# Jarvis73/PEMP

Hardware: AMD Instinct MI355X
Metric: episodes/sec (PEMP stage-1 eval step, PASCAL-5i-shaped 1-shot, ResNet-50) (higher is better)
Workload: dtype f32

## Files before the change

include/pemp_hip.h:

```cpp
#ifndef PEMP_HIP_H
#define PEMP_HIP_H

#include <stddef.h>
#include <stdint.h>

#ifdef __cplusplus
extern "C" {
#endif

#define PEMP_ABI_VERSION 2

#define PEMP_CONV_RELU 1u
#define PEMP_CONV_SHIFT_PER_IMAGE 2u
#define PEMP_CONV_STEM4 4u
#define PEMP_CONV_POOL3S2 8u
#define PEMP_CONV_OUT_SPLIT3 16u
#define PEMP_CONV_IN_SPLIT3 32u
#define PEMP_CONV_OUT_SPLIT3_ALSO 64u

typedef struct pemp_conv_desc {
    int32_t N, H, W;
    int32_t Cin, ldx;
    int32_t Ho, Wo;
    int32_t Cout, ldy;
// ... 13 lines not shown
int pemp_conv2d_nhwc_f32(const pemp_conv_desc* d, const float* x, const float* w, float* y,
                         const float* scale, const float* shift, const float* residual,
                         void* stream);

int pemp_conv2d_padv_nhwc_f32(const pemp_conv_desc* d, const float* x, const float* w, float* y,
                              const float* scale, const float* shift, const float* residual,
                              const float* pad_value, void* stream);

int pemp_conv2d_hybrid_rows(const pemp_conv_desc* d);

int pemp_conv2d_group_nhwc_f32(int n, const pemp_conv_desc* d, const float* const* x, const float* const* w,
                               float* const* y, const float* const* scale, const float* const* shift,
                               const float* const* residual, const float* const* pad_value, void* stream);

int pemp_pack_split3_bf16(const float* w, void* out, int cout, int kpad, void* stream);

int pemp_conv2d_bf16_nhwc(const pemp_conv_desc* d, const void* x, const void* w, void* y, const float* scale,
                          const float* shift, const void* residual, const void* pad_value, int out_f32, void* stream);
int pemp_convert_f32_bf16(const float* x, void* y, long long n, void* stream);
int pemp_convert_bf16_f32(const void* x, float* y, long long n, void* stream);

int pemp_conv2d_dropblock_nhwc_f32(const pemp_conv_desc* d, const float* x, const float* w, float* y, const float* scale,
                                   const float* shift, const float* residual, const float* rowmask, const int* kept_count,
                                   void* ws, size_t ws_bytes, void* stream);
int pemp_bn_apply_dropblock_f32(const float* z, int ldz, const float* mean, const float* invstd, const float* gamma,
                                const float* beta, float* y, int ldy, int M, int C, const float* rowmask,
                                const int* kept_count, void* stream);

int pemp_pack_input_nhwc4_f32(const float* img, const float* prior, float* out,
                              int N, int H, int W, void* stream);
// ... 254 lines not shown
```

pemp_amd/_lib.py:

```python
import ctypes as C
import os

import torch

_HERE = os.path.dirname(os.path.abspath(__file__))
LIB_PATH = os.environ.get("PEMP_HIP_LIB", os.path.join(_HERE, "libpemp_hip.so"))

c_fp = C.c_void_p
c_int = C.c_int
c_size = C.c_size_t


class ConvDesc(C.Structure):
    _fields_ = [(n, C.c_int32) for n in
                ("N", "H", "W", "Cin", "ldx", "Ho", "Wo", "Cout", "ldy", "KH", "KW",
                 "stride", "pad", "dil", "ldr", "Kpad")] + [("flags", C.c_uint32), ("tile", C.c_int32)]


class SampleDesc(C.Structure):
    _fields_ = [("img_off", C.c_int64), ("msk_off", C.c_int64), ("img_out", C.c_int64), ("msk_out", C.c_int64)] + \
               [(n, C.c_int32) for n in ("hs", "ws", "sh", "sw", "oy", "ox", "flip", "jitter_order")] + \
               [("jitter", C.c_float * 3), ("mask_mode", C.c_int32), ("ksx", C.c_int32), ("ksy", C.c_int32),
                ("ws_off", C.c_int64)]

# ... 5 lines not shown
CONV_OUT_SPLIT3 = 16
CONV_IN_SPLIT3 = 32
CONV_OUT_SPLIT3_ALSO = 64

SYMBOLS = {
    "pemp_last_error": (C.c_char_p, []),
    "pemp_abi_version": (c_int, []),
    "pemp_conv2d_hybrid_rows": (c_int, [C.POINTER(ConvDesc)]),
    "pemp_conv2d_tile_shape": (c_int, [c_int, C.POINTER(c_int), C.POINTER(c_int)]),
    "pemp_conv2d_nhwc_f32": (c_int, [C.POINTER(ConvDesc), c_fp, c_fp, c_fp, c_fp, c_fp, c_fp, c_fp]),
    "pemp_conv2d_padv_splitk_nhwc_f32": (c_int, [C.POINTER(ConvDesc), c_fp, c_fp, c_fp, c_fp, c_fp, c_fp, c_fp, c_fp, c_size, c_fp]),
    "pemp_conv2d_padv_nhwc_f32": (c_int, [C.POINTER(ConvDesc), c_fp, c_fp, c_fp, c_fp, c_fp, c_fp, c_fp, c_fp]),
    "pemp_conv2d_group_nhwc_f32": (c_int, [c_int, C.POINTER(ConvDesc)] + [C.POINTER(c_fp)] * 7 + [c_fp]),
    "pemp_conv2d_bf16_nhwc": (c_int, [C.POINTER(ConvDesc), c_fp, c_fp, c_fp, c_fp, c_fp, c_fp, c_fp, c_int, c_fp]),
    "pemp_pack_split3_bf16": (c_int, [c_fp, c_fp, c_int, c_int, c_fp]),
    "pemp_convert_f32_bf16": (c_int, [c_fp, c_fp, C.c_longlong, c_fp]),
    "pemp_convert_bf16_f32": (c_int, [c_fp, c_fp, C.c_longlong, c_fp]),
    "pemp_conv2d_dropblock_nhwc_f32": (c_int, [C.POINTER(ConvDesc), c_fp, c_fp, c_fp, c_fp, c_fp, c_fp, c_fp, c_fp, c_fp, c_size, c_fp]),
    "pemp_bn_apply_dropblock_f32": (c_int, [c_fp, c_int, c_fp, c_fp, c_fp, c_fp, c_fp, c_int, c_int, c_int, c_fp, c_fp, c_fp]),
    "pemp_pack_input_nhwc4_f32": (c_int, [c_fp, c_fp, c_fp, c_int, c_int, c_int, c_fp]),
    "pemp_maxpool2d_nhwc_f32": (c_int, [c_fp, c_fp] + [c_int] * 11 + [c_fp]),
    "pemp_global_avgpool_nhwc_f32": (c_int, [c_fp, c_fp, c_int, c_int, c_int, c_int, c_fp]),
    "pemp_channel_affine_multi_f32": (c_int, [c_fp, c_int, c_int, c_int, c_int,
                                              C.POINTER(c_fp), C.POINTER(c_fp), C.POINTER(c_fp),
                                              C.POINTER(c_int), c_fp]),
    "pemp_mpm_workspace_bytes": (c_size, [c_int] * 5),
    "pemp_mpm_protos_f32": (c_int, [c_fp, c_int, c_fp, c_fp, c_fp, c_fp, c_size] + [c_int] * 8 + [c_fp]),
    "pemp_map_workspace_bytes": (c_size, [c_int] * 4),
    "pemp_masked_avg_pool_f32": (c_int, [c_fp, c_int, c_fp, c_fp, c_fp, c_size] + [c_int] * 8 + [c_fp]),
    "pemp_cosine_proto_max_f32": (c_int, [c_fp, c_int, c_fp, c_fp, c_fp, c_int, c_int, c_int, c_int,
# ... 140 lines not shown
```

pemp_amd/csrc/conv_common.h:

```cpp
#pragma once
#include "common.h"

namespace pemp {

typedef __attribute__((ext_vector_type(16))) float f32x16;
typedef __attribute__((ext_vector_type(4))) float v4f;
typedef __attribute__((ext_vector_type(8))) __bf16 bf16x8;
typedef __attribute__((ext_vector_type(2))) unsigned int u32x2;

#define PEMP_CONV_BF16_IO 0x100u

__device__ __forceinline__ v4f load_quad(const float* base, size_t off, unsigned bf16) {
    if (!bf16) return *(const v4f*)(base + off);
    const u32x2 r = *(const u32x2*)((const unsigned short*)base + off);
    return v4f{__builtin_bit_cast(float, r.x << 16), __builtin_bit_cast(float, r.x & 0xFFFF0000u),
               __builtin_bit_cast(float, r.y << 16), __builtin_bit_cast(float, r.y & 0xFFFF0000u)};
}

__device__ __forceinline__ unsigned int bf16_bits(float f) {
    const unsigned int u = __builtin_bit_cast(unsigned int, f);
    if ((u & 0x7FFFFFFFu) > 0x7F800000u) return (u >> 16) | 0x40u;
    return (u + 0x7FFFu + ((u >> 16) & 1u)) >> 16;
}

// ... 300 lines not shown
int conv_dma2_hybrid_rows(int M, int Cout);
int launch_conv_dma2_bf16(int shape, const ConvArgs& a, hipStream_t st);
int launch_conv_dma2_db(int shape, ConvArgs a, void* ws, size_t ws_bytes, bool split, hipStream_t st);
struct SplitKPlan { int full, split, pieces; size_t ws_bytes; };
SplitKPlan conv_dma2_splitk_plan(int shape, const ConvArgs& a);
int launch_conv_dma2_splitk(int shape, ConvArgs a, void* ws, size_t ws_bytes, hipStream_t st);
int launch_conv_dma2_split3(int shape, ConvArgs a, void* ws, size_t ws_bytes, bool split, hipStream_t st);
int launch_conv_dma2_group_split3(int shape, ConvGroupArgs& g, hipStream_t st);
int launch_conv_dma2_split3_stats(int shape, const ConvArgs& a, hipStream_t st);
bool conv_dma2_split3_stats_shape(int shape);
int launch_conv_dma2_split3_persist(int shape, const ConvArgs& a, hipStream_t st);
bool conv_dma2_persist_out_split3(int shape);
int launch_conv_dma2_split3_pre(int shape, bool persistent, const ConvArgs& a, hipStream_t st);
bool conv_panel_supported(const ConvArgs& a);
int launch_conv_panel(int shape, const ConvArgs& a, hipStream_t st);
int conv_dma2_simds();
int pack_split3(const float* w, void* out, int cout, int kpad, hipStream_t st);
int launch_conv_stem_pool(const ConvArgs& a, hipStream_t st);
int conv_stem_pool_out(int i);

}
```

pemp_amd/csrc/conv_igemm.hip:

```cpp
#include "conv_tiles.h"

namespace pemp {


template <int BM, int BN, int WGM, bool STEM>
__global__ __launch_bounds__(256) void conv_igemm_kernel(ConvArgs a) {
    constexpr int WGN = 4 / WGM;
    constexpr int WM = BM / WGM, WN = BN / WGN;
    constexpr int TM = WM / 32, TN = WN / 32;
    constexpr int AL = BM / 32, BL = BN / 32;
    static_assert(TM >= 1 && TN >= 1, "wave tile");

    extern __shared__ __attribute__((aligned(16))) v4f smem[];
    v4f* As = smem;
    v4f* Bs = smem + 2 * 8 * BM;

    const int tid = threadIdx.x;
    const int lane = tid & 63;
    const int wave = tid >> 6;
    const int wm0 = (wave / WGN) * WM;
    const int wn0 = (wave % WGN) * WN;
    const int lr = lane & 31, lh = lane >> 5;

    const int ntn = a.Cout / BN;
// ... 336 lines not shown
        if (conv_dma2_supported(a)) {
            PEMP_REQUIRE_COUT("conv2d", t.shape, a.Cout);
            return launch_conv_dma2(t.shape, a, st);
        }
        t.family = TILE_DMA;
        if (t.shape == 8) t.shape = 3;
    }
    if (t.family == TILE_DMA) {
        PEMP_REQUIRE_COUT("conv2d", t.shape, a.Cout);
        return launch_conv_dma(t.shape, a, st);
    }
    PEMP_REQUIRE(t.shape != 1 || a.Cout % 128 == 0, "conv2d: tile 128x128 needs Cout %% 128 == 0");
    return launch_conv(t.shape, a, st);
}


extern "C" int pemp_conv2d_group_nhwc_f32(int n, const pemp_conv_desc* d, const float* const* x, const float* const* w,
                                          float* const* y, const float* const* scale, const float* const* shift,
                                          const float* const* residual, const float* const* pad_value, void* stream) {
    PEMP_REQUIRE(n >= 1 && n <= CONV_GROUP_MAX && d && x && w && y, "conv2d_group: 1..%d member convs", CONV_GROUP_MAX);
    ConvGroupArgs g;
    g.n = n;
    const int tile = d[0].tile;
    const TileId t = decode_tile(tile);
    const bool s3 = t.family == TILE_SPLIT3 && t.exists && !t.splitk && !t.persistent && !t.panel && !t.presplit;
    PEMP_REQUIRE((t.family == TILE_DMA2 && !t.splitk && t.shape <= 8) || s3, "conv2d_group: tile must be one of the buffer-addressed variants 21..28 or 41..44, 46, got %d", tile);
    for (int i = 0; i < n; ++i) {
        PEMP_REQUIRE(d[i].tile == tile, "conv2d_group: every member must name the same tile variant");
        PEMP_REQUIRE(!pad_value || (pad_value[i] != nullptr) == (pad_value[0] != nullptr), "conv2d_group: pad_value for every member or for none");
        const int rc = conv_fill(&d[i], x[i], w[i], y[i], scale ? scale[i] : nullptr, shift ? shift[i] : nullptr,
// ... 208 lines not shown
```

pemp_amd/csrc/conv_panel.hip:

```cpp
#include "conv_tiles.h"

namespace pemp {

typedef __attribute__((address_space(3))) void* lptr_t;
typedef __attribute__((ext_vector_type(4))) unsigned int v4u;

template <int NK> constexpr bool panel_early() { return NK >= 4; }
template <int NK, int BN> constexpr bool panel_two_blocks() { return BN == 64 && NK <= 4; }
template <int NK, int BN> constexpr int panel_stages() {
    if (!panel_early<NK>()) return 3;
    if (NK == 4) return 5;
    return BN == 64 ? 8 : 6;
}
template <int NK, int NS, int BL, int NST>
constexpr int panel_behind(int kt) {
    int c = 0;
    for (int u = kt + 1 - NS; u <= kt - 1; ++u) {
        const int ku = ((u % NK) + NK) % NK;
        if (u > kt + 1 - NS) c += BL;
        if (ku == NK - 1) c += NST;
    }
    return c;
}
template <int NK, int NS, int BL, int NST>
constexpr int panel_behind_max() {
    int m = 0;
    for (int kt = 0; kt < NK; ++kt) m = panel_behind<NK, NS, BL, NST>(kt) > m ? panel_behind<NK, NS, BL, NST>(kt) : m;
    return m;
}
template <int NK, int NS, int BL, int NST, int KT = 0>
__device__ __forceinline__ void panel_wait(int kt) {
    if constexpr (KT < NK) {
        if (kt == KT) asm volatile("s_waitcnt vmcnt(%0) lgkmcnt(0)" ::"n"(panel_behind<NK, NS, BL, NST>(KT)) : "memory");
        else panel_wait<NK, NS, BL, NST, KT + 1>(kt);
    }
}

template <int NK, int BN, int NW>
// ... 217 lines not shown
#undef PEMP_PANEL_AFFINE
#undef PEMP_PANEL_READ
#undef PEMP_PANEL_MMA_HOOKED
#undef PEMP_PANEL_HOOK_NONE
#undef PEMP_PANEL_HOOK_DMA
#undef PEMP_PANEL_HOOK_DMA_RES
#undef PEMP_PANEL_MMA
#endif
}

template <int NK, int BN, int NW>
__global__ __launch_bounds__(NW * 64) __attribute__((amdgpu_waves_per_eu(panel_two_blocks<NK, BN>() ? 2 : 1))) void conv_panel_kernel(ConvArgs a) {
    conv_panel_body<NK, BN, NW>(a);
}

constexpr int PANEL_NW = 4;
template <int NK, int BN> constexpr size_t panel_lds() { return (size_t)(panel_stages<NK, BN>() * BN * 12 + PANEL_NW * 256) * sizeof(v4f); }
static_assert(panel_lds<8, 128>() <= 160 * 1024 && 2 * panel_lds<4, 64>() <= 160 * 1024, "LDS of a CU");

template <int BN, int NK = 1>
static int launch_panel_nk(const ConvArgs& a, hipStream_t st) {
    if constexpr (NK > 8) {
        set_error("conv split3 panel: Kpad=%d above 256", a.Kpad);
        return -1;
    } else {
        if (a.nk == NK)
            return launch_with_lds(conv_panel_kernel<NK, BN, PANEL_NW>, cdiv(a.M, 32 * PANEL_NW), PANEL_NW * 64, panel_lds<NK, BN>(), st, a,
                                   "conv_panel");
        return launch_panel_nk<BN, NK + 1>(a, st);
    }
// ... 4 lines not shown
        return false;
    if (a.padv || a.stats || a.rowmask || a.sk_S > 1 || a.bm_first) return false;
    const long long lim = 1ll << 31;
    return (long long)a.N * a.H * a.W * a.ldx * 4 < lim && (long long)a.M * a.ldy * 4 < lim && (!a.res || (long long)a.M * a.ldr * 4 < lim) &&
           (long long)a.Cout * a.Kpad * 6 < lim;
}

int launch_conv_panel(int shape, const ConvArgs& a, hipStream_t st) {
    if (!conv_panel_supported(a)) {
        set_error("conv split3 panel: needs a 1x1 conv without padding, Kpad <= 256, no padding value / per-image shift, operands < 2 GiB");
        return -1;
    }
    return kTileShapes[shape].bn == 128 ? launch_panel_nk<128>(a, st) : launch_panel_nk<64>(a, st);
}

}
```

pemp_amd/engine.py:

```python
import os

import torch
import torch.nn as nn

from . import ops
from .ops import ConvParams

BN_EPS = 1e-5

SPLIT3 = os.environ.get("PEMP_SPLIT3", "1") != "0"


def split3_admits(cp):
    return (cp.w.dtype == torch.float32 and not cp.stem and cp.kh * cp.kw <= 32 and cp.cin % 32 == 0 and cp.cout % 64 == 0
            and cp.kpad == cp.kh * cp.kw * cp.cin)


def with_split3(cp):
    if not SPLIT3 or cp.w.dtype != torch.float32:
        return cp
    if cp.stem:
        if (cp.kh, cp.kw, cp.stride, cp.pad, cp.dil) == (7, 7, 2, 3, 1) and cp.kpad == 224 and cp.cout % 64 == 0:
            cp.w3pool = ops.pack_split3(cp.w)
    elif split3_admits(cp):
# ... 105 lines not shown
        if extra_in:
            sl = (0, blk.conv1.weight.shape[1] - extra_in)
        self.c1 = conv_params(blk.conv1, blk.bn1, relu=True, in_slice=sl, dtype=dtype)
        self.c2 = conv_params(blk.conv2, blk.bn2, relu=True, dtype=dtype)
        self.c3 = conv_params(blk.conv3, blk.bn3, relu=True, dtype=dtype)
        self.ds = conv_params(blk.downsample[0], blk.downsample[1], relu=False, in_slice=sl, dtype=dtype) \
            if blk.downsample is not None else None
        if extra_in:
            self.c1_extra = (blk.conv1.weight.detach()[:, sl[1]:, 0, 0].float() * self.c1.scale[:, None]).contiguous()
            self.ds_extra = (blk.downsample[0].weight.detach()[:, sl[1]:, 0, 0].float() * self.ds.scale[:, None]).contiguous()


class _BottleneckTrunk:
    GROUP_DS = True
    PRESPLIT = True

    def _block(self, x, bp, tag, c1_shift=None, ds_shift=None, out=None):
        a = self.arena
        n, h, w, _ = x.shape
        h1, w1 = (ops.conv_out_size(v, k, bp.c1.stride, bp.c1.pad, bp.c1.dil) for v, k in ((h, bp.c1.kh), (w, bp.c1.kw)))
        ho, wo = (ops.conv_out_size(v, k, bp.c2.stride, bp.c2.pad, bp.c2.dil) for v, k in ((h1, bp.c2.kh), (w1, bp.c2.kw)))
        if out is None:
            out = a.get(("blk", tag), (n, ho, wo, bp.c3.cout))
        res = a.get("res", (n, ho, wo, bp.ds.cout)) if bp.ds is not None else x
        grouped = self.GROUP_DS and bp.ds is not None and c1_shift is None and ds_shift is None \
            and 0 < n * ho * wo <= GROUP_MAX_ROWS and x.dtype == torch.float32
        pre = presplit_pair(bp.c1, bp.c2, x, n * ho * wo, self.PRESPLIT and not grouped)
        y1 = a.get("y1s", ops.split3_shape(n, h1, w1, bp.c1.cout), torch.bfloat16) if pre else a.get("y1", (n, h1, w1, bp.c1.cout))
        if grouped:
            ops.conv2d_group([x, x], [bp.c1, bp.ds], [y1, res])
        else:
            ops.conv2d(x, bp.c1, out=y1, shift_override=c1_shift, per_image_shift=c1_shift is not None, out_split3=pre)
        y2 = ops.conv2d(y1, bp.c2, out=a.get("y2", (n, ho, wo, bp.c2.cout)), x_split3=pre)
        if bp.ds is not None and not grouped:
            ops.conv2d(x, bp.ds, out=res, shift_override=ds_shift, per_image_shift=ds_shift is not None)
        return ops.conv2d(y2, bp.c3, out=out, residual=res)

    def _stage(self, x, si, final_out=None):
        blocks = self.stages[si]
        for bi, bp in enumerate(blocks):
            x = self._block(x, bp, (si, bi & 1), out=final_out if bi == len(blocks) - 1 else None)
        return x


class ResNetEngine(_BottleneckTrunk):

    def __init__(self, prm, arena):
        self.arena = arena
        self.stem = conv_params(prm.conv1, prm.bn1, relu=True, stem4=True)
        self.stages = []
        for name in ("layer1", "layer2", "layer3"):
            self.stages.append([_BlockPlan(b, dtype=arena.dtype) for b in getattr(prm, name)])

    def stem_forward(self, x4):
        a = self.arena
        n, h, w, _ = x4.shape
# ... 261 lines not shown
```

pemp_amd/ops.py:

```python
import ctypes as C
import collections
import functools
import json
import os

import torch

from . import _lib
from ._lib import ConvDesc, CONV_RELU, CONV_SHIFT_PER_IMAGE, CONV_STEM4, CONV_POOL3S2, CONV_OUT_SPLIT3, CONV_IN_SPLIT3, CONV_OUT_SPLIT3_ALSO


def _stream():
    return C.c_void_p(torch.cuda.current_stream().cuda_stream)


def _p(t):
    return C.c_void_p(t.data_ptr()) if t is not None else C.c_void_p(0)


def _chk_dev(*ts):
    for t in ts:
        if t is not None and (not t.is_cuda):
            raise _lib.PempHipError("pemp_amd ops need device (cuda/HIP) tensors; there is no CPU path")

# ... 358 lines not shown
                key += (71,)
            cands = lambda: _fits(list(SPLIT3_TILES) + (list(SPLIT3_SPLITK_TILES) if splitk else []) +
                                  (list(SPLIT3_PANEL_TILES) if panel else []), p.cout)
        else:
            def cands():
                ids = list(GROUP_TILES if dropblock is not None else TILE_VARIANTS) + (list(SPLITK_TILES) if splitk else [])
                if 29 in ids and not (hybrid_rows(n, ho, wo, p.cout) and dma2_supported(x, p)):
                    ids.remove(29)
                return _fits(ids, p.cout)
        tile = _choose_tile(key, n * ho * wo, launch, cands,
                            SPLIT3_PRESPLIT_TILES[0] if x_split3 else SPLIT3_DEFAULT_TILE if s3 else DEFAULT_TILE + (10 if dropblock is not None else 0))
    launch(tile)
    return out


def stem_pool_supported(p):
    return (p.stem and p.w3pool is not None and (p.kh, p.kw, p.stride, p.pad, p.dil) == (7, 7, 2, 3, 1) and p.kpad == 224
            and p.cout % 64 == 0)


def stem_pool(x, p, out=None):
    lib = _lib.load()
    if not stem_pool_supported(p):
        raise ValueError("stem_pool: a 7x7 / stride 2 / pad 3 NHWC4 stem with split weights (ConvParams.w3pool)")
    _chk_dev(x, p.w3pool, out)
    ldx = _nhwc(x, "x")
    n, h, w, cin = x.shape
    if cin != p.cin or x.dtype != torch.float32:
        raise ValueError(f"stem_pool: fp32 NHWC4 input expected, got {cin} channels of {x.dtype}")
    ho, wo = conv_out_size(h, 7, 2, 3, 1), conv_out_size(w, 7, 2, 3, 1)
# ... 801 lines not shown
```

pemp_amd/pfenet_engine.py:

```python
import torch

from . import ops
from .engine import _BlockPlan, _BottleneckTrunk, classifier2, conv_params, logits_nchw, pack_episode, with_split3
from .ops import ConvParams

PYRAMID_BINS = (60, 30, 15, 8)
REDUCE = 256
MERGE_CIN = REDUCE + 32


class DeepBaseResNetEngine(_BottleneckTrunk):
    PRESPLIT = False
    GROUP_DS = False

    def __init__(self, model, arena):
        self.arena = arena
        l0 = model.layer0
        self.stem = [conv_params(l0[0], l0[1], relu=True, stem4=True), conv_params(l0[3], l0[4], relu=True),
                     conv_params(l0[6], l0[7], relu=True)]
        self.stages = [[_BlockPlan(b) for b in getattr(model, f"layer{i}")] for i in (1, 2, 3, 4)]

    def forward_to_layer3(self, x4):
        a = self.arena
        n, H, W, _ = x4.shape
        x = x4
        for i, cp in enumerate(self.stem):
            h, w = x.shape[1:3]
            ho, wo = ops.conv_out_size(h, 3, cp.stride, cp.pad, 1), ops.conv_out_size(w, 3, cp.stride, cp.pad, 1)
# ... 93 lines not shown
```

Measured before the change: 1465.

## Fuse bottleneck conv3 with downsample conv and next block's conv1 in panel kernel

Adds a panel-chain kernel that computes a bottleneck's final 1x1 conv together with the downsample 1x1 conv (as a second K source), and optionally the next block's 1x1 conv1 (C1=64) from the fresh output tile. This is meant to remove separate launches and the round trips of the residual and block output through global memory. The trunk's stage loop is rewritten to hand the next block's y1 across blocks. An autotuner picks fused or sequential execution per shape, which adds tuning overhead and extra register and LDS pressure.

Measured after the change: 1484, median of 6. 1.3% higher.

```diff
diff --git a/include/pemp_hip.h b/include/pemp_hip.h
--- a/include/pemp_hip.h
+++ b/include/pemp_hip.h
@@ -51,6 +51,12 @@
                                const float* const* residual, const float* const* pad_value, void* stream);
 
 int pemp_pack_split3_bf16(const float* w, void* out, int cout, int kpad, void* stream);
+
+int pemp_split3_panel_chain_nhwc_f32(const pemp_conv_desc* d, const float* x, const void* w3, float* y, const float* scale,
+                                     const float* shift, const float* residual, const pemp_conv_desc* d_ds, const float* x_ds,
+                                     const void* w3_ds, const float* scale_ds, const float* shift_ds, const void* w3_c1,
+                                     const float* scale_c1, const float* shift_c1, float* y1, int c1, int ldy1,
+                                     unsigned flags_c1, void* stream);
 
 int pemp_conv2d_bf16_nhwc(const pemp_conv_desc* d, const void* x, const void* w, void* y, const float* scale,
                           const float* shift, const void* residual, const void* pad_value, int out_f32, void* stream);
diff --git a/pemp_amd/_lib.py b/pemp_amd/_lib.py
--- a/pemp_amd/_lib.py
+++ b/pemp_amd/_lib.py
@@ -43,6 +43,8 @@
     "pemp_conv2d_group_nhwc_f32": (c_int, [c_int, C.POINTER(ConvDesc)] + [C.POINTER(c_fp)] * 7 + [c_fp]),
     "pemp_conv2d_bf16_nhwc": (c_int, [C.POINTER(ConvDesc), c_fp, c_fp, c_fp, c_fp, c_fp, c_fp, c_fp, c_int, c_fp]),
     "pemp_pack_split3_bf16": (c_int, [c_fp, c_fp, c_int, c_int, c_fp]),
+    "pemp_split3_panel_chain_nhwc_f32": (c_int, [C.POINTER(ConvDesc)] + [c_fp] * 6 + [C.POINTER(ConvDesc)] + [c_fp] * 8
+                                         + [c_int, c_int, C.c_uint32, c_fp]),
     "pemp_convert_f32_bf16": (c_int, [c_fp, c_fp, C.c_longlong, c_fp]),
     "pemp_convert_bf16_f32": (c_int, [c_fp, c_fp, C.c_longlong, c_fp]),
     "pemp_conv2d_dropblock_nhwc_f32": (c_int, [C.POINTER(ConvDesc), c_fp, c_fp, c_fp, c_fp, c_fp, c_fp, c_fp, c_fp, c_fp, c_size, c_fp]),
diff --git a/pemp_amd/csrc/conv_common.h b/pemp_amd/csrc/conv_common.h
--- a/pemp_amd/csrc/conv_common.h
+++ b/pemp_amd/csrc/conv_common.h
@@ -338,6 +338,16 @@
 int launch_conv_dma2_split3_pre(int shape, bool persistent, const ConvArgs& a, hipStream_t st);
 bool conv_panel_supported(const ConvArgs& a);
 int launch_conv_panel(int shape, const ConvArgs& a, hipStream_t st);
+struct PanelChainArgs {
+    ConvArgs a;
+    const float *xd, *wd, *scd, *shd;
+    int ldxd;
+    const float *w1, *sc1, *sh1;
+    float* y1;
+    int ldy1, relu1;
+};
+bool conv_panel_chain_instantiated(int kpad, int ds_channels, int c1);
+int launch_conv_panel_chain(const PanelChainArgs& g, int ds_channels, bool ch, hipStream_t st);
 int conv_dma2_simds();
 int pack_split3(const float* w, void* out, int cout, int kpad, hipStream_t st);
 int launch_conv_stem_pool(const ConvArgs& a, hipStream_t st);
diff --git a/pemp_amd/csrc/conv_igemm.hip b/pemp_amd/csrc/conv_igemm.hip
--- a/pemp_amd/csrc/conv_igemm.hip
+++ b/pemp_amd/csrc/conv_igemm.hip
@@ -374,6 +374,68 @@
     return launch_conv(t.shape, a, st);
 }
 
+extern "C" int pemp_split3_panel_chain_nhwc_f32(const pemp_conv_desc* d, const float* x, const void* w3, float* y, const float* scale,
+                                                const float* shift, const float* residual, const pemp_conv_desc* d_ds,
+                                                const float* x_ds, const void* w3_ds, const float* scale_ds, const float* shift_ds,
+                                                const void* w3_c1, const float* scale_c1, const float* shift_c1, float* y1, int c1,
+                                                int ldy1, unsigned flags_c1, void* stream) {
+    const char* who = "split3_panel_chain";
+    PanelChainArgs g = {};
+    PEMP_REQUIRE(d && (d->tile == 0 || d->tile == 72), "%s: tile id 72 (or 0) only: no split-K, workspace or other form", who);
+    PEMP_REQUIRE(!(d->flags & ~PEMP_CONV_RELU), "%s: no per-image shift, stem, pooled or pre-split form (flags 0x%x)", who, d->flags);
+    int rc = conv_fill(d, x, (const float*)w3, y, scale, shift, residual, nullptr, g.a);
+    if (rc) return rc;
+    PEMP_REQUIRE(g.a.KH == 1 && g.a.KW == 1 && g.a.pad == 0, "%s: a 1x1 conv without padding", who);
+    PEMP_REQUIRE(g.a.Kpad <= 256, "%s: Kpad=%d above 256", who, g.a.Kpad);
+    PEMP_REQUIRE(conv_panel_supported(g.a), "%s: operands past the 2 GiB window of a buffer descriptor", who);
+    const bool ds = d_ds || x_ds || w3_ds, ch = w3_c1 || y1 || c1;
+    const long long M = g.a.M;
+    int dsc = 0;
+    if (ds) {
+        ConvArgs ad;
+        PEMP_REQUIRE(d_ds && x_ds && w3_ds, "%s: the second source needs its descriptor, tensor and packed weights", who);
+        PEMP_REQUIRE(!residual, "%s: a second source stands where the residual would: not both", who);
+        PEMP_REQUIRE(d_ds->flags == 0 && (d_ds->tile == 0 || d_ds->tile == 72), "%s: the second source is a plain conv (no ReLU, no flags, no tile id)", who);
+        rc = conv_fill(d_ds, x_ds, (const float*)w3_ds, y, scale_ds, shift_ds, nullptr, nullptr, ad);
+        if (rc) return rc;
+        PEMP_REQUIRE(ad.KH == 1 && ad.KW == 1 && ad.pad == 0 && ad.stride == 1, "%s: the second source is a 1x1 conv of stride 1 without padding", who);
+        PEMP_REQUIRE(ad.M == g.a.M && ad.Cout == g.a.Cout, "%s: the second source has %d rows x %d channels of output, the conv %d x %d", who, ad.M,
+                     ad.Cout, g.a.M, g.a.Cout);
+        PEMP_REQUIRE(ad.Cin <= 128, "%s: the second source has %d channels, at most 128", who, ad.Cin);
+        PEMP_REQUIRE(M * ad.ldx * 4 < (1ll << 31), "%s: operands past the 2 GiB window of a buffer descriptor", who);
+        g.xd = x_ds, g.wd = (const float*)w3_ds, g.scd = scale_ds, g.shd = shift_ds, g.ldxd = ad.ldx;
+        dsc = ad.Cin;
+    }
+    if (ch) {
+        PEMP_REQUIRE(w3_c1 && y1, "%s: the chained conv needs its packed weights and its output", who);
+        PEMP_REQUIRE(c1 == 64, "%s: the chained conv is built for C1 = 64, got %d", who, c1);
+        PEMP_REQUIRE(ldy1 >= c1 && ldy1 % 4 == 0 && ((uintptr_t)y1 & 15) == 0 && ((uintptr_t)w3_c1 & 15) == 0,
+                     "%s: ldy1 must be >= C1 and a multiple of 4, y1 and its weights 16-byte aligned", who);
+        PEMP_REQUIRE((!scale_c1 || ((uintptr_t)scale_c1 & 15) == 0) && (!shift_c1 || ((uintptr_t)shift_c1 & 15) == 0), "%s: scale / shift must be 16-byte aligned", who);
+        PEMP_REQUIRE(!(flags_c1 & ~PEMP_CONV_RELU), "%s: the chained conv takes PEMP_CONV_RELU only", who);
+        PEMP_REQUIRE(M * ldy1 * 4 < (1ll << 31), "%s: operands past the 2 GiB window of a buffer descriptor", who);
+        g.w1 = (const float*)w3_c1, g.sc1 = scale_c1, g.sh1 = shift_c1, g.y1 = y1, g.ldy1 = ldy1, g.relu1 = (flags_c1 & PEMP_CONV_RELU) ? 1 : 0;
+    }
+    auto clash = [](const void* pa, long long rows_a, int ld_a, int c_a, const void* pb, long long rows_b, int ld_b, int c_b) {
+        if (!pa || !pb) return false;
+        const char *a0 = (const char*)pa, *a1 = a0 + ((rows_a - 1) * ld_a + c_a) * 4;
+        const char *b0 = (const char*)pb, *b1 = b0 + ((rows_b - 1) * ld_b + c_b) * 4;
+        return a0 < b1 && b0 < a1;
+    };
+    const long long rows_x = (long long)g.a.N * g.a.H * g.a.W;
+    PEMP_REQUIRE(!clash(y, M, g.a.ldy, g.a.Cout, x, rows_x, g.a.ldx, g.a.Cin) && !clash(y, M, g.a.ldy, g.a.Cout, residual, M, g.a.ldr, g.a.Cout) &&
+                     !clash(y, M, g.a.ldy, g.a.Cout, x_ds, M, g.ldxd, dsc),
+                 "%s: y overlaps an input", who);
+    PEMP_REQUIRE(!clash(y1, M, ldy1, c1, x, rows_x, g.a.ldx, g.a.Cin) && !clash(y1, M, ldy1, c1, residual, M, g.a.ldr, g.a.Cout) &&
+                     !clash(y1, M, ldy1, c1, x_ds, M, g.ldxd, dsc),
+                 "%s: y1 overlaps an input", who);
+    PEMP_REQUIRE(!clash(y, M, g.a.ldy, g.a.Cout, y1, M, ldy1, c1), "%s: y and y1 overlap", who);
+    if (!ds && !ch) return launch_conv_panel(2, g.a, (hipStream_t)stream);
+    PEMP_REQUIRE(conv_panel_chain_instantiated(g.a.Kpad, dsc, ch ? c1 : 0),
+                 "%s: built for Kpad = 64 (got %d), a second source of 32 / 64 / 128 channels (got %d), C1 = 64", who, g.a.Kpad, dsc);
+    return launch_conv_panel_chain(g, dsc, ch, (hipStream_t)stream);
+}
+
 
 extern "C" int pemp_conv2d_group_nhwc_f32(int n, const pemp_conv_desc* d, const float* const* x, const float* const* w,
                                           float* const* y, const float* const* scale, const float* const* shift,
diff --git a/pemp_amd/csrc/conv_panel.hip b/pemp_amd/csrc/conv_panel.hip
--- a/pemp_amd/csrc/conv_panel.hip
+++ b/pemp_amd/csrc/conv_panel.hip
@@ -12,16 +12,18 @@
     if (NK == 4) return 5;
     return BN == 64 ? 8 : 6;
 }
+template <int P, int PE, int NS, int BL, int NST>
+constexpr int panel_seq_behind(int p) {
+    int c = 0;
+    for (int u = p + 1 - NS; u <= p - 1; ++u) {
+        const int pu = ((u % P) + P) % P;
+        if (u > p + 1 - NS) c += BL;
+        if (pu == PE - 1) c += NST;
+    }
+    return c;
+}
 template <int NK, int NS, int BL, int NST>
-constexpr int panel_behind(int kt) {
-    int c = 0;
-    for (int u = kt + 1 - NS; u <= kt - 1; ++u) {
-        const int ku = ((u % NK) + NK) % NK;
-        if (u > kt + 1 - NS) c += BL;
-        if (ku == NK - 1) c += NST;
-    }
-    return c;
-}
+constexpr int panel_behind(int kt) { return panel_seq_behind<NK, NK, NS, BL, NST>(kt); }
 template <int NK, int NS, int BL, int NST>
 constexpr int panel_behind_max() {
     int m = 0;
@@ -269,6 +271,330 @@
     conv_panel_body<NK, BN, NW>(a);
 }
 
+template <int P, int PE, int NS, int BL, int NST, int Q = 0>
+__device__ __forceinline__ void panel_seq_wait(int p) {
+    if constexpr (Q < P) {
+        if (p == Q) asm volatile("s_waitcnt vmcnt(%0) lgkmcnt(0)" ::"n"(panel_seq_behind<P, PE, NS, BL, NST>(Q)) : "memory");
+        else panel_seq_wait<P, PE, NS, BL, NST, Q + 1>(p);
+    }
+}
+template <int NKD> constexpr int panel_chain_stages() { return 3; }
+template <int P, int PE, int NS, int BL, int NST>
+constexpr int panel_seq_behind_max() {
+    int m = 0;
+    for (int p = 0; p < P; ++p) m = panel_seq_behind<P, PE, NS, BL, NST>(p) > m ? panel_seq_behind<P, PE, NS, BL, NST>(p) : m;
+    return m;
+}
+template <int P, int PE, int NS, int BL, int NST>
+constexpr int panel_seq_behind_sum() {
+    int c = 0;
+    for (int p = 0; p < P; ++p) c += panel_seq_behind<P, PE, NS, BL, NST>(p);
+    return c;
+}
+
+template <int NK, int NKD, bool CH, int BN, int NW>
+__device__ __forceinline__ void conv_panel_chain_body(const PanelChainArgs& g) {
+#if defined(__HIP_DEVICE_COMPILE__)
+    const ConvArgs& a = g.a;
+    constexpr bool DS = NKD > 0;
+    constexpr int TN = BN / 32;
+    constexpr int SQ = BN * 12;
+    static_assert(SQ % (NW * 64) == 0, "whole DMA rounds");
+    constexpr int BL = SQ / (NW * 64);
+    constexpr int NST = TN * 4;
+    constexpr int NS = panel_chain_stages<NKD>();
+    constexpr int NKC = CH ? BN / 32 : 0;
+    constexpr int PE = NK + NKD;
+    constexpr int P = PE + NKC;
+    constexpr int NP = 1 + (DS ? 1 : 0) + (CH ? 1 : 0);
+    static_assert(DS || CH, "the plain form is conv_panel_kernel");
+    static_assert(!CH || BN == 64, "a W1 stage has the 64 rows of a W3 stage: C1 == BN == 64");
+    static_assert(panel_seq_behind_max<P, PE, NS, BL, NST>() <= 63, "vmcnt range");
+    static_assert(panel_seq_behind<P, PE, NS, BL, NST>(PE % P) >= (NS - 2) * BL + NST &&
+                      panel_seq_behind_sum<P, PE, NS, BL, NST>() == P * (NS - 2) * BL + (NS - 1) * NST,
+                  "NS - 2 DMAs in every window; a tile's stores in the windows of the NS - 1 steps behind its epilogue");
+
+    extern __shared__ __attribute__((aligned(16))) v4f smem[];
+    v4f* Bs = smem;
+    const int tid = threadIdx.x;
+    const int lane = tid & 63;
+    const int wave = __builtin_amdgcn_readfirstlane(tid >> 6);
+    float* patch = (float*)(smem + NS * SQ) + wave * (1024 * NP);
+    float* patch_d = patch + 1024;
+    float* patch_o = patch + (DS ? 2048 : 1024);
+    const int lr = lane & 31, lh = lane >> 5;
+    const int m_wave = ((int)blockIdx.x * NW + wave) * 32;
+    const int ntn = a.Cout / BN;
+
+    const __amdgpu_buffer_rsrc_t rx = __builtin_amdgcn_make_buffer_rsrc((void*)a.x, 0, 0x80000000u, 0x00020000);
+    const __amdgpu_buffer_rsrc_t rw = __builtin_amdgcn_make_buffer_rsrc((void*)a.w, 0, 0x80000000u, 0x00020000);
+    const __amdgpu_buffer_rsrc_t ry = __builtin_amdgcn_make_buffer_rsrc((void*)a.y, 0, 0x80000000u, 0x00020000);
+    const __amdgpu_buffer_rsrc_t rr = __builtin_amdgcn_make_buffer_rsrc((void*)(a.res ? a.res : a.y), 0, 0x80000000u, 0x00020000);
+    const __amdgpu_buffer_rsrc_t rxd = __builtin_amdgcn_make_buffer_rsrc((void*)(DS ? g.xd : a.x), 0, 0x80000000u, 0x00020000);
+    const __amdgpu_buffer_rsrc_t rwd = __builtin_amdgcn_make_buffer_rsrc((void*)(DS ? g.wd : a.w), 0, 0x80000000u, 0x00020000);
+    const __amdgpu_buffer_rsrc_t rw1 = __builtin_amdgcn_make_buffer_rsrc((void*)(CH ? g.w1 : a.w), 0, 0x80000000u, 0x00020000);
+    const __amdgpu_buffer_rsrc_t ry1 = __builtin_amdgcn_make_buffer_rsrc((void*)(CH ? g.y1 : a.y), 0, 0x80000000u, 0x00020000);
+
+    unsigned b_voff[BL], b_voffd[BL], b_voff1[BL];
+#pragma unroll
+    for (int i = 0; i < BL; ++i) {
+        const int q = i * NW * 64 + tid, row = q / 12, pos = q - row * 12;
+        const int src = (pos & ~3) | ((pos & 3) ^ ((row >> 2) & 3));
+        b_voff[i] = (unsigned)(row * a.Kpad * 6 + src * 16);
+        b_voffd[i] = (unsigned)(row * (NKD * 32) * 6 + src * 16);
+        b_voff1[i] = (unsigned)(row * a.Cout * 6 + src * 16);
+    }
+    auto dma = [&](int buf_, int n_, int p_) __attribute__((always_inline)) {
+        v4f* const Bd_ = Bs + buf_ * SQ + wave * 64;
+        const bool in_ = n_ < ntn;
+        if (p_ < NK) {
+            const int so_ = __builtin_amdgcn_readfirstlane(in_ ? n_ * BN * a.Kpad * 6 + p_ * 192 : 0);
+#pragma unroll
+            for (int i = 0; i < BL; ++i)
+                __builtin_amdgcn_raw_ptr_buffer_load_lds(rw, (lptr_t)(Bd_ + i * NW * 64), 16, in_ ? b_voff[i] : 0x80000000u, so_, 0, 0);
+        } else if (p_ < PE) {
+            const int so_ = __builtin_amdgcn_readfirstlane(in_ ? n_ * BN * (NKD * 32) * 6 + (p_ - NK) * 192 : 0);
+#pragma unroll
+            for (int i = 0; i < BL; ++i)
+                __builtin_amdgcn_raw_ptr_buffer_load_lds(rwd, (lptr_t)(Bd_ + i * NW * 64), 16, in_ ? b_voffd[i] : 0x80000000u, so_, 0, 0);
+        } else {
+            const int so_ = __builtin_amdgcn_readfirstlane(in_ ? (n_ * NKC + p_ - PE) * 192 : 0);
+#pragma unroll
+            for (int i = 0; i < BL; ++i)
+                __builtin_amdgcn_raw_ptr_buffer_load_lds(rw1, (lptr_t)(Bd_ + i * NW * 64), 16, in_ ? b_voff1[i] : 0x80000000u, so_, 0, 0);
+        }
+    };
+
+#pragma unroll
+    for (int t = 0; t < NS; ++t) dma(t, t / P, t % P);
+
+    bf16x8 ah[2 * NK], am[2 * NK], al[2 * NK];
+    bf16x8 dh[DS ? 2 * NKD : 1], dm[DS ? 2 * NKD : 1], dl[DS ? 2 * NKD : 1];
+    {
+        const int m = m_wave + lr;
+        const bool ok = m < a.M;
+        const int mm = ok ? m : 0;
+        const int img = mm / a.HoWo;
+        const int rem = mm - img * a.HoWo;
+        const int ho = rem / a.Wo;
+        const int wo = rem - ho * a.Wo;
+        const unsigned off = ok ? (unsigned)(((img * a.H + ho * a.stride) * a.W + wo * a.stride) * a.ldx + 8 * lh) * 4u : 0x80000000u;
+        const unsigned offd = ok ? (unsigned)(mm * g.ldxd + 8 * lh) * 4u : 0x80000000u;
+        v4f x0[2 * NK], x1[2 * NK], d0[DS ? 2 * NKD : 1], d1[DS ? 2 * NKD : 1];
+#pragma unroll
+        for (int s = 0; s < 2 * NK; ++s) {
+            x0[s] = __builtin_bit_cast(v4f, __builtin_amdgcn_raw_buffer_load_b128(rx, off + s * 64, 0, 0));
+            x1[s] = __builtin_bit_cast(v4f, __builtin_amdgcn_raw_buffer_load_b128(rx, off + s * 64 + 16, 0, 0));
+        }
+        if constexpr (DS) {
+#pragma unroll
+            for (int s = 0; s < 2 * NKD; ++s) {
+                d0[s] = __builtin_bit_cast(v4f, __builtin_amdgcn_raw_buffer_load_b128(rxd, offd + s * 64, 0, 0));
+                d1[s] = __builtin_bit_cast(v4f, __builtin_amdgcn_raw_buffer_load_b128(rxd, offd + s * 64 + 16, 0, 0));
+            }
+        }
+#pragma unroll
+        for (int s = 0; s < 2 * NK; ++s) split3_bf16(x0[s], x1[s], ah[s], am[s], al[s]);
+        if constexpr (DS) {
+#pragma unroll
+            for (int s = 0; s < 2 * NKD; ++s) split3_bf16(d0[s], d1[s], dh[s], dm[s], dl[s]);
+        }
+    }
+    asm volatile("s_waitcnt vmcnt(0)" ::: "memory");
+    __builtin_amdgcn_s_barrier();
+    __builtin_amdgcn_sched_barrier(0);
+
+    const int brow3 = lr * 12, bsw3 = (lr >> 2) & 3;
+    v4f bfr[2][TN][3];
+    auto read_b = [&](int dst_, int buf_, int j_) __attribute__((always_inline)) {
+        const v4f* Bb_ = Bs + buf_ * SQ;
+        const int pb_ = (2 * j_ + lh) ^ bsw3;
+#pragma unroll
+        for (int ni = 0; ni < TN; ++ni)
+#pragma unroll
+            for (int pl = 0; pl < 3; ++pl) bfr[dst_][ni][pl] = Bb_[brow3 + ni * 32 * 12 + pl * 4 + pb_];
+    };
+    auto mma = [&](int src_, const bf16x8& h_, const bf16x8& m_, const bf16x8& l_, f32x16 (&c_)[TN]) __attribute__((always_inline)) {
+#pragma unroll
+        for (int pr = 0; pr < 6; ++pr)
+#pragma unroll
+            for (int ni = 0; ni < TN; ++ni) {
+                const bf16x8 av_ = pr == 0 ? l_ : (pr == 2 || pr == 3) ? m_ : h_;
+                const bf16x8 bv_ = __builtin_bit_cast(bf16x8, bfr[src_][ni][pr == 1 ? 2 : (pr == 2 || pr == 4) ? 1 : 0]);
+                c_[ni] = __builtin_amdgcn_mfma_f32_32x32x16_bf16(av_, bv_, c_[ni], 0, 0, 0);
+            }
+    };
+
+    f32x16 acc[TN], accd[DS ? TN : 1], acc1[CH ? TN : 1];
+    bf16x8 ch[CH ? 2 * TN : 1], cm[CH ? 2 * TN : 1], cl[CH ? 2 * TN : 1];
+#pragma unroll
+    for (int ni = 0; ni < TN; ++ni)
+#pragma unroll
+        for (int e = 0; e < 16; ++e) {
+            acc[ni][e] = 0.f;
+            if constexpr (DS) accd[ni][e] = 0.f;
+            if constexpr (CH) acc1[ni][e] = 0.f;
+        }
+    auto step_mma = [&](int src_, int p_, int j_) __attribute__((always_inline)) {
+        if (p_ < NK) mma(src_, ah[2 * p_ + j_], am[2 * p_ + j_], al[2 * p_ + j_], acc);
+        else if (p_ < PE) {
+            if constexpr (DS) mma(src_, dh[2 * (p_ - NK) + j_], dm[2 * (p_ - NK) + j_], dl[2 * (p_ - NK) + j_], accd);
+        } else {
+            if constexpr (CH) mma(src_, ch[2 * (p_ - PE) + j_], cm[2 * (p_ - PE) + j_], cl[2 * (p_ - PE) + j_], acc1);
+        }
+    };
+
+    const bool relu = a.flags & PEMP_CONV_RELU;
+    const int er = lane >> 3, c4 = (lane & 7) * 4;
+    unsigned y_off[4], r_off[4], y1_off[4];
+#pragma unroll
+    for (int i = 0; i < 4; ++i) {
+        const int m = m_wave + er + 8 * i;
+        y_off[i] = m < a.M ? (unsigned)(m * a.ldy + c4) * 4u : 0x80000000u;
+        r_off[i] = m < a.M ? (unsigned)(m * a.ldr + c4) * 4u : 0x80000000u;
+        y1_off[i] = m < a.M ? (unsigned)(m * g.ldy1 + c4) * 4u : 0x80000000u;
+    }
+    auto affine = [&](const float* sc_, const float* sh_, int c_, v4f& scq_, v4f& shq_) __attribute__((always_inline)) {
+        scq_ = sc_ ? *(const v4f*)(sc_ + c_) : v4f{1.f, 1.f, 1.f, 1.f};
+        shq_ = sh_ ? *(const v4f*)(sh_ + c_) : v4f{0.f, 0.f, 0.f, 0.f};
+    };
+    auto to_patch = [&](float* S_, const f32x16& c_) __attribute__((always_inline)) {
+#pragma unroll
+        for (int e = 0; e < 16; ++e) S_[((e & 3) + 8 * (e >> 2) + 4 * lh) * 32 + lr] = c_[e];
+    };
+
+    int cur = 0;
+    read_b(0, 0, 0);
+    for (int n = 0; n < ntn; ++n) {
+        v4f rres[NST], scv[TN], shv[TN], scdv[TN], shdv[TN];
+#pragma unroll
+        for (int p = 0; p < P; ++p) {
+            const int nxt = cur == NS - 1 ? 0 : cur + 1;
+            read_b(1, cur, 1);
+            __builtin_amdgcn_sched_barrier(0);
+            step_mma(0, p, 0);
+            __builtin_amdgcn_sched_barrier(0);
+            panel_seq_wait<P, PE, NS, BL, NST>(p);
+            __builtin_amdgcn_s_barrier();
+            __builtin_amdgcn_sched_barrier(0);
+            read_b(0, nxt, 0);
+            if (p == PE - 1) {
+#pragma unroll
+                for (int ni = 0; ni < TN; ++ni) {
+                    affine(a.scale, a.shift, n * BN + ni * 32 + c4, scv[ni], shv[ni]);
+                    if constexpr (DS) affine(g.scd, g.shd, n * BN + ni * 32 + c4, scdv[ni], shdv[ni]);
+                }
+                if constexpr (!DS) {
+#pragma unroll
+                    for (int i = 0; i < NST; ++i) rres[i] = v4f{0.f, 0.f, 0.f, 0.f};
+                    if (a.res) {
+#pragma unroll
+                        for (int ni = 0; ni < TN; ++ni)
+#pragma unroll
+                            for (int i = 0; i < 4; ++i)
+                                rres[ni * 4 + i] = __builtin_bit_cast(v4f, __builtin_amdgcn_raw_buffer_load_b128(rr, r_off[i] + (unsigned)(n * BN + ni * 32) * 4u, 0, 0));
+                    }
+                }
+            }
+            __builtin_amdgcn_sched_barrier(0);
+            dma(cur, n + (p + NS) / P, (p + NS) % P);
+            __builtin_amdgcn_sched_barrier(0);
+            step_mma(1, p, 1);
+            __builtin_amdgcn_sched_barrier(0);
+            cur = nxt;
+            if (p == PE - 1) {
+#pragma unroll
+                for (int ni = 0; ni < TN; ++ni) {
+                    const v4f sc = scv[ni], sh = shv[ni];
+                    to_patch(patch, acc[ni]);
+                    if constexpr (DS) to_patch(patch_d, accd[ni]);
+                    asm volatile("s_waitcnt lgkmcnt(0)" ::: "memory");
+#pragma unroll
+                    for (int i = 0; i < 4; ++i) {
+                        const int row = er + 8 * i;
+                        const v4f v = *(const v4f*)(patch + row * 32 + c4);
+                        v4f add = sh;
+                        if constexpr (DS) {
+                            const v4f vd = *(const v4f*)(patch_d + row * 32 + c4);
+                            v4f r;
+                            r.x = __builtin_fmaf(vd.x, scdv[ni].x, shdv[ni].x);
+                            r.y = __builtin_fmaf(vd.y, scdv[ni].y, shdv[ni].y);
+                            r.z = __builtin_fmaf(vd.z, scdv[ni].z, shdv[ni].z);
+                            r.w = __builtin_fmaf(vd.w, scdv[ni].w, shdv[ni].w);
+                            add += r;
+                        } else {
+                            if (a.res) add += rres[ni * 4 + i];
+                        }
+                        v4f o;
+                        o.x = __builtin_fmaf(v.x, sc.x, add.x);
+                        o.y = __builtin_fmaf(v.y, sc.y, add.y);
+                        o.z = __builtin_fmaf(v.z, sc.z, add.z);
+                        o.w = __builtin_fmaf(v.w, sc.w, add.w);
+                        if (relu) {
+                            o.x = fmaxf(o.x, 0.f);
+                            o.y = fmaxf(o.y, 0.f);
+                            o.z = fmaxf(o.z, 0.f);
+                            o.w = fmaxf(o.w, 0.f);
+                        }
+                        __builtin_amdgcn_raw_buffer_store_b128(__builtin_bit_cast(v4u, o), ry, y_off[i] + (unsigned)(n * BN + ni * 32) * 4u, 0, 0);
+                        if constexpr (CH) *(v4f*)(patch_o + row * 32 + (((lane & 7) ^ ((row >> 1) & 7)) << 2)) = o;
+                    }
+                    if constexpr (CH) {
+                        asm volatile("s_waitcnt lgkmcnt(0)" ::: "memory");
+                        const int sw = (lr >> 1) & 7;
+#pragma unroll
+                        for (int s = 0; s < 2; ++s) {
+                            const v4f o0 = *(const v4f*)(patch_o + lr * 32 + (((4 * s + 2 * lh) ^ sw) << 2));
+                            const v4f o1 = *(const v4f*)(patch_o + lr * 32 + (((4 * s + 2 * lh + 1) ^ sw) << 2));
+                            split3_bf16(o0, o1, ch[2 * ni + s], cm[2 * ni + s], cl[2 * ni + s]);
+                        }
+                    }
+                    asm volatile("s_waitcnt lgkmcnt(0)" ::: "memory");
+#pragma unroll
+                    for (int e = 0; e < 16; ++e) {
+                        acc[ni][e] = 0.f;
+                        if constexpr (DS) accd[ni][e] = 0.f;
+                    }
+                }
+                __builtin_amdgcn_sched_barrier(0);
+            }
+        }
+    }
+    if constexpr (CH) {
+#pragma unroll
+        for (int ni = 0; ni < TN; ++ni) {
+            v4f sc, sh;
+            affine(g.sc1, g.sh1, ni * 32 + c4, sc, sh);
+            to_patch(patch, acc1[ni]);
+            asm volatile("s_waitcnt lgkmcnt(0)" ::: "memory");
+#pragma unroll
+            for (int i = 0; i < 4; ++i) {
+                const v4f v = *(const v4f*)(patch + (er + 8 * i) * 32 + c4);
+                v4f o;
+                o.x = __builtin_fmaf(v.x, sc.x, sh.x);
+                o.y = __builtin_fmaf(v.y, sc.y, sh.y);
+                o.z = __builtin_fmaf(v.z, sc.z, sh.z);
+                o.w = __builtin_fmaf(v.w, sc.w, sh.w);
+                if (g.relu1) {
+                    o.x = fmaxf(o.x, 0.f);
+                    o.y = fmaxf(o.y, 0.f);
+                    o.z = fmaxf(o.z, 0.f);
+                    o.w = fmaxf(o.w, 0.f);
+                }
+                __builtin_amdgcn_raw_buffer_store_b128(__builtin_bit_cast(v4u, o), ry1, y1_off[i] + (unsigned)(ni * 32) * 4u, 0, 0);
+            }
+            asm volatile("s_waitcnt lgkmcnt(0)" ::: "memory");
+        }
+    }
+    asm volatile("s_waitcnt vmcnt(0)" ::: "memory");
+#endif
+}
+
+template <int NK, int NKD, bool CH, int BN, int NW>
+__global__ __launch_bounds__(NW * 64) __attribute__((amdgpu_waves_per_eu(1))) void conv_panel_chain_kernel(PanelChainArgs g) {
+    conv_panel_chain_body<NK, NKD, CH, BN, NW>(g);
+}
+
 constexpr int PANEL_NW = 4;
 template <int NK, int BN> constexpr size_t panel_lds() { return (size_t)(panel_stages<NK, BN>() * BN * 12 + PANEL_NW * 256) * sizeof(v4f); }
 static_assert(panel_lds<8, 128>() <= 160 * 1024 && 2 * panel_lds<4, 64>() <= 160 * 1024, "LDS of a CU");
@@ -303,4 +629,26 @@
     return kTileShapes[shape].bn == 128 ? launch_panel_nk<128>(a, st) : launch_panel_nk<64>(a, st);
 }
 
-}
+template <int NKD, bool CH>
+static int launch_panel_chain(const PanelChainArgs& g, hipStream_t st) {
+    constexpr int NP = 1 + (NKD > 0 ? 1 : 0) + (CH ? 1 : 0);
+    constexpr size_t lds = (size_t)(panel_chain_stages<NKD>() * 64 * 12 + PANEL_NW * 256 * NP) * sizeof(v4f);
+    static_assert(lds <= 160 * 1024, "LDS of a CU");
+    return launch_with_lds(conv_panel_chain_kernel<2, NKD, CH, 64, PANEL_NW>, cdiv(g.a.M, 32 * PANEL_NW), PANEL_NW * 64, lds, st, g, "conv_panel_chain");
+}
+
+bool conv_panel_chain_instantiated(int kpad, int ds_channels, int c1) {
+    if (kpad != 64 || (c1 != 0 && c1 != 64)) return false;
+    return c1 ? ds_channels == 0 || ds_channels == 64 : ds_channels == 32 || ds_channels == 64 || ds_channels == 128;
+}
+
+int launch_conv_panel_chain(const PanelChainArgs& g, int ds_channels, bool ch, hipStream_t st) {
+    if (!conv_panel_supported(g.a) || !conv_panel_chain_instantiated(g.a.Kpad, ds_channels, ch ? 64 : 0)) {
+        set_error("conv split3 panel chain: needs conv_panel's geometry at Kpad = 64 with a second source of 32 / 64 / 128 channels or C1 = 64 (with 0 / 64)");
+        return -1;
+    }
+    if (ch) return ds_channels ? launch_panel_chain<2, true>(g, st) : launch_panel_chain<0, true>(g, st);
+    return ds_channels == 32 ? launch_panel_chain<1, false>(g, st) : ds_channels == 64 ? launch_panel_chain<2, false>(g, st) : launch_panel_chain<4, false>(g, st);
+}
+
+}
diff --git a/pemp_amd/engine.py b/pemp_amd/engine.py
--- a/pemp_amd/engine.py
+++ b/pemp_amd/engine.py
@@ -143,6 +143,7 @@
 class _BottleneckTrunk:
     GROUP_DS = True
     PRESPLIT = True
+    CHAIN = True
 
     def _block(self, x, bp, tag, c1_shift=None, ds_shift=None, out=None):
         a = self.arena
@@ -165,10 +166,39 @@
             ops.conv2d(x, bp.ds, out=res, shift_override=ds_shift, per_image_shift=ds_shift is not None)
         return ops.conv2d(y2, bp.c3, out=out, residual=res)
 
+    def _hands_over(self, x, bp, nbp):
+        if not (self.CHAIN and nbp is not None and nbp.ds is None and self.arena.dtype == torch.float32 and x.dtype == torch.float32):
+            return False
+        n, h, w, _ = x.shape
+        if bp.c1.stride != 1 or bp.c2.stride != 1 or n * h * w <= GROUP_MAX_ROWS or presplit_pair(nbp.c1, nbp.c2, x, n * h * w, self.PRESPLIT):
+            return False
+        y2 = self.arena.get("y2", (n, h, w, bp.c2.cout))
+        return ops.chain_supported(y2, bp.c3, None, (x, bp.ds) if bp.ds is not None else None, nbp.c1)
+
+    def _block_chained(self, x, bp, tag, y1, nbp, out=None):
+        a = self.arena
+        n, h, w, _ = x.shape
+        if out is None:
+            out = a.get(("blk", tag), (n, h, w, bp.c3.cout))
+        if y1 is None:
+            y1 = ops.conv2d(x, bp.c1, out=a.get("y1", (n, h, w, bp.c1.cout)))
+        y2 = ops.conv2d(y1, bp.c2, out=a.get("y2", (n, h, w, bp.c2.cout)))
+        ds = (x, bp.ds, lambda: a.get("res", (n, h, w, bp.ds.cout))) if bp.ds is not None else None
+        y1n = a.get("y1", (n, h, w, nbp.c1.cout)) if nbp is not None else None
+        ops.conv3_chain(y2, bp.c3, out, residual=None if ds else x, ds=ds, nxt=(nbp.c1, y1n) if nbp is not None else None)
+        return out, y1n
+
     def _stage(self, x, si, final_out=None):
         blocks = self.stages[si]
+        y1 = None
         for bi, bp in enumerate(blocks):
-            x = self._block(x, bp, (si, bi & 1), out=final_out if bi == len(blocks) - 1 else None)
+            last = bi == len(blocks) - 1
+            out = final_out if last else None
+            hand = not last and self._hands_over(x, bp, blocks[bi + 1])
+            if hand or y1 is not None:
+                x, y1 = self._block_chained(x, bp, (si, bi & 1), y1, blocks[bi + 1] if hand else None, out)
+            else:
+                x = self._block(x, bp, (si, bi & 1), out=out)
         return x
 
 
diff --git a/pemp_amd/ops.py b/pemp_amd/ops.py
--- a/pemp_amd/ops.py
+++ b/pemp_amd/ops.py
@@ -396,6 +396,82 @@
     return out
 
 
+PANEL_CHAIN = os.environ.get("PEMP_PANEL_CHAIN", "1") != "0"
+PANEL_CHAIN_FORCE = None
+PANEL_CHAIN_FORMS = {(True, True): True, (False, True): True, (True, False): True}
+
+
+def _is_1x1s1(p):
+    return p.kh == 1 and p.kw == 1 and p.stride == 1 and p.pad == 0 and p.w3 is not None and not p.stem
+
+
+def chain_supported(y2, c3, residual=None, ds=None, nxt=None):
+    if not (PANEL_CHAIN and PICK_HOOK is None and y2.is_cuda and y2.dtype == torch.float32 and y2.dim() == 4 and _is_1x1s1(c3)
+            and c3.kpad == 64 and c3.cin == 64 and c3.cout % 64 == 0 and (ds is not None or nxt is not None)):
+        return False
+    rows = y2.shape[0] * y2.shape[1] * y2.shape[2]
+    if rows * max(c3.cout, y2.stride(2) if y2.shape[2] > 1 else c3.cin) * 4 >= 2 ** 31:
+        return False
+    if ds is not None:
+        x, dp = ds
+        if not (residual is None and _is_1x1s1(dp) and dp.cout == c3.cout and not dp.relu and x.dtype == torch.float32 and x.dim() == 4
+                and tuple(x.shape[:3]) == tuple(y2.shape[:3]) and dp.cin == (64 if nxt is not None else dp.cin) and dp.cin in (32, 64, 128)
+                and x.numel() * 4 < 2 ** 31):
+            return False
+    return nxt is None or (_is_1x1s1(nxt) and nxt.cin == c3.cout and nxt.cout == 64)
+
+
+def conv3_chain(y2, c3, out, residual=None, ds=None, nxt=None):
+    dsx, dsp, res_buf = ds if ds is not None else (None, None, None)
+    c1, y1 = nxt if nxt is not None else (None, None)
+    if ds is not None and residual is not None:
+        raise ValueError("conv3_chain: a downsample conv stands where the residual would: not both")
+
+    def sequence():
+        r = residual
+        if ds is not None:
+            r = conv2d(dsx, dsp, out=res_buf() if callable(res_buf) else res_buf)
+        conv2d(y2, c3, out=out, residual=r)
+        if nxt is not None:
+            conv2d(out, c1, out=y1)
+
+    if not chain_supported(y2, c3, residual, (dsx, dsp) if ds is not None else None, c1):
+        sequence()
+        return out
+    n, h, w, cin, ldx, ho, wo, out, ldy, ldr = _conv_geom("conv3_chain", y2, c3, out, residual)
+    lib = _lib.load()
+    _chk_dev(y2, out, residual, dsx, y1)
+    d = ConvDesc(n, h, w, cin, ldx, ho, wo, c3.cout, ldy, 1, 1, 1, 0, 1, ldr, c3.kpad, CONV_RELU if c3.relu else 0, 72)
+    dd = None
+    if ds is not None:
+        ldxd = _nhwc(dsx, "ds x")
+        dd = ConvDesc(n, h, w, dsp.cin, ldxd, ho, wo, dsp.cout, dsp.cout, 1, 1, 1, 0, 1, 0, dsp.kpad, 0, 72)
+    ldy1 = 0
+    if nxt is not None:
+        ldy1 = _nhwc(y1, "y1")
+        if tuple(y1.shape) != (n, ho, wo, c1.cout):
+            raise ValueError(f"conv3_chain: y1 shape {tuple(y1.shape)} != {(n, ho, wo, c1.cout)}")
+
+    def fused():
+        _lib.check(lib.pemp_split3_panel_chain_nhwc_f32(
+            C.byref(d), _p(y2), _p(c3.w3), _p(out), _p(c3.scale), _p(c3.shift), _p(residual),
+            C.byref(dd) if dd is not None else None, _p(dsx), _p(dsp.w3 if dsp else None), _p(dsp.scale if dsp else None),
+            _p(dsp.shift if dsp else None), _p(c1.w3 if c1 else None), _p(c1.scale if c1 else None), _p(c1.shift if c1 else None),
+            _p(y1), c1.cout if c1 else 0, ldy1, CONV_RELU if (c1 and c1.relu) else 0, _stream()), "pemp_split3_panel_chain_nhwc_f32")
+
+    if PANEL_CHAIN_FORCE is not None:
+        pick = int(PANEL_CHAIN_FORCE)
+    else:
+        key = (7200, c3.cin, c3.cout, dsp.cin if dsp else 0, c1.cout if c1 else 0, n, h, w, int(residual is not None))
+        pick = _TILE_CACHE.get(key)
+        if pick is None:
+            pick = 0
+            if PANEL_CHAIN_FORMS.get((ds is not None, nxt is not None)) and _tunes(n * ho * wo):
+                pick = _pick_tile(lambda f: fused() if f else sequence(), key, [0, 1])
+    fused() if pick else sequence()
+    return out
+
+
 def stem_pool_supported(p):
     return (p.stem and p.w3pool is not None and (p.kh, p.kw, p.stride, p.pad, p.dil) == (7, 7, 2, 3, 1) and p.kpad == 224
             and p.cout % 64 == 0)
diff --git a/pemp_amd/pfenet_engine.py b/pemp_amd/pfenet_engine.py
--- a/pemp_amd/pfenet_engine.py
+++ b/pemp_amd/pfenet_engine.py
@@ -12,6 +12,7 @@
 class DeepBaseResNetEngine(_BottleneckTrunk):
     PRESPLIT = False
     GROUP_DS = False
+    CHAIN = False
 
     def __init__(self, model, arena):
         self.arena = arena
```
